# mjrgh/DCSExplorer

Hardware: AMD Instinct MI355X
Metric: bit_exact_int16_pcm_samples_per_sec (higher is better)
Workload: dtype int16; 1 GPU; survey3_65536; gpu_max_hw_queues=4, samples_per_frame=240, frames_per_wave=8, wavefronts_per_launch=8192, arithmetic=ADSP-2105 1.15 fixed point, 32-bit integer intermediates, partition=range over streams, no collective, scale=1, inflight=1, frames_per_chunk=all, full=False

## Files before the change

### dcsexplorer_amd/csrc/dcs_decode_chunk.inc.h

```cpp
    DCS_STAMP(1);

    struct { uint32_t job; uint32_t prevSlot, flags, nSrc, shiftXform; uint32_t firstSrc, prevJob, poolOff, bpl; } slot;
    uint32_t exportNext;
    uint4 pd0, pd1, phdr;
    uint2 pd2;
    uint32_t planHdr0 = 0, planHdr1 = 0, planType0 = 0, planType1 = 0;
    {
        uint4 *scratch = reinterpret_cast<uint4 *>(L.pool());
        static_assert(kHeadVec * 16 <= poolDwords(FPW) * 4, "the package head fits in the bit pool");
        if (lane < kHeadVec)
            scratch[lane] = phead0;
        if (kHeadLoads > 1 && lane + 64 < kHeadVec)
            scratch[lane + 64] = phead1;
        waveSync();
        const uint4 *sp5 = scratch + 5 * s;
        const uint4 s0 = sp5[0];
        pd0 = sp5[1]; pd1 = sp5[2];
        const uint4 d2v = sp5[3];
        pd2 = make_uint2(d2v.x, d2v.y);
        phdr = sp5[4];
        if constexpr (bandPlanInLds(FPW))
        {
            const unsigned char *bytes = reinterpret_cast<const unsigned char *>(sp5) + q;
            planType0 = bytes[36]; planType1 = bytes[44];
// ... 166 lines not shown
                const uint32_t hw = static_cast<uint32_t>((streamOff + 2) >> 2);
                const uint32_t sh = static_cast<uint32_t>((streamOff + 2) & 3);
                uint32_t hdrW[5];
#pragma unroll
                for (int i = 0 ; i < 5 ; ++i)
                    hdrW[i] = (has && hw + i < blobWords) ? blobW[hw + i] : 0u;
                Q.h0 = __builtin_amdgcn_alignbyte(hdrW[1], hdrW[0], sh);
                Q.h1 = __builtin_amdgcn_alignbyte(hdrW[2], hdrW[1], sh);
                Q.h2 = __builtin_amdgcn_alignbyte(hdrW[3], hdrW[2], sh);
                Q.h3 = __builtin_amdgcn_alignbyte(hdrW[4], hdrW[3], sh);
                if (hdrLen == 1)
                {
                    Q.h0 &= 0xFFu; Q.h1 = Q.h2 = Q.h3 = 0;
                }
            }
            waveSync();

            if (R0) DCS_STAMP(3);
            const bool ok = has && fits && unpacker;
            if (has && !fits && q == 0)
                err |= DCS_FRAME_FATAL | DCS_FRAME_STOP;
            if (has && q == 0)
                err |= flags >> 4;
            uint32_t relBits = hdrBits;
            Q.bandBase = 0;
            Q.outIdx = 1;
            Q.prv = 0; Q.prvDelta = 0;
            Q.subType = (format == DCS_FMT_93B_T1) ? 0 : 2;
            Q.reuse = false; Q.first = true;
            Q.midEnd = Q.midStart = Q.midStraddle = false;
            Q.endIdx = 0;
            constexpr bool evenDeal = R0 && SUB == 8 && EVEN;
            if (serial)
                Q.nb = (q == 0) ? nBands : 0;
            else
            {
                const int nb16 = min(nBands, 16);
                if (R0)
                {
                    const bool f93a = format == DCS_FMT_93A_T1;
                    const int nbEnd = f93a ? min(nBands, 18) : nb16;
                    const int myBase = (sp.x & 0x8000u) ? nbEnd
                                     : static_cast<int>(sp.y >> 28) + ((f93a && (sp.y & (DCS_SPLIT_BASE16 << 16)) != 0) ? 16 : 0);
                    const int nextBase = __shfl(myBase, lane + FPW);
                    Q.bandBase = myBase;
                    Q.nb = max((q == SUB - 1 ? nbEnd : nextBase) - myBase, 0);
                    if (SUB == 16)
                    {
                        const bool mid = format >= DCS_FMT_94_T0 && q == SUB - 1 && myBase == 15 && (sp.y & (DCS_SPLIT_MID15 << 16)) != 0;
                        const bool nextMid = __shfl(static_cast<int>(mid), lane + FPW) != 0;
                        Q.midStart = mid;
                        Q.midStraddle = mid && (sp.y & (DCS_MID15_STRADDLE << 16)) != 0;
                        Q.midEnd = q == SUB - 2 && nextMid;
                        if (Q.midEnd)
                            Q.nb = 16 - myBase;
                    }
                    if constexpr (evenDeal)
                    {
                        const bool mid = format >= DCS_FMT_94_T0 && !(sp.x & 0x8000u) && (sp.y & (DCS_SPLIT_MID15 << 16)) != 0;
                        const bool nextMid = __shfl(static_cast<int>(mid), lane + FPW) != 0 && q != SUB - 1;
                        const int nextIdx = __shfl(static_cast<int>((sp.y >> 16) & 0x1FFu), lane + FPW);
                        Q.midStart = mid;
                        Q.midStraddle = mid && (sp.y & (DCS_MID15_STRADDLE << 16)) != 0;
                        Q.midEnd = nextMid;
                        Q.endIdx = nextIdx;
                        if (nextMid)
                            Q.nb = min(nextBase + 1, nbEnd) - myBase;
                    }
                }
                else
                {
                    const int bpl = max((nb16 + SUB - 1) / SUB, 1);
                    if (format == DCS_FMT_93A_T1)
                    {
                        Q.bandBase = min(q * bpl, nb16);
                        Q.nb = min(max(nb16 - Q.bandBase, 0), bpl);
                    }
                    else
                    {
                        Q.bandBase = dcsLaneFirstBand(format, q, bpl, nb16);
                        Q.nb = (q == SUB - 1 ? nb16 : dcsLaneFirstBand(format, q + 1, bpl, nb16)) - Q.bandBase;
                    }
                }
                if (q != 0 && Q.nb != 0)
                {
                    if (!R0)
                        sp = reinterpret_cast<const uint2 *>(sdp)[5 + Q.bandBase - 1];
                    const uint32_t sp0 = sp.x, sp1 = sp.y;
                    relBits = sp0 & 0x7FFFu;
                    Q.prv = sp0 >> 16;
                    Q.prvDelta = sp1 & 0xFFFFu;
                    const uint32_t st = sp1 >> 16;
                    Q.outIdx = static_cast<int>(st & 0x1FFu);
                    Q.subType = static_cast<int>((st >> 9) & 3u);
                    Q.reuse = (st & 0x800u) != 0;
                    Q.first = false;
                }
            }
            const uint32_t inPool = static_cast<uint32_t>(bitPos & 31) + relBits;
            const uint32_t *brAt = pool + (ok ? off + (inPool >> 5) : 0u);
            const int brBit = static_cast<int>(inPool & 31);

            if (R0) DCS_STAMP(12);
            const bool is94 = ok && format >= DCS_FMT_94_T0;
            const bool is93a = ok && format == DCS_FMT_93A_T1 && Q.nb != 0 && !(Q.bandBase != 0 && Q.reuse);
            const bool is93 = ok && format < DCS_FMT_93A_T1;
            if (__any(is94))
            {
                BR94 br;
                br.init(brAt, brBit);
                const uint32_t planAt = (R0 && bandPlanInLds(FPW))
                    ? static_cast<uint32_t>(reinterpret_cast<uintptr_t>((LdsBytePtr)L.plan())) + static_cast<uint32_t>(Q.bandBase * FPW + s) * kPlanRecBytes
                    : 0u;
                err |= unpack94<R0, BR94, SUB, evenDeal>(T, row, br, Q, format, mixMul, is94, stamp, planAt);
            }
            if constexpr (!SOLE)
            {
            BR93 br;
            br.init(brAt, brBit);
            if (__any(is93))
                err |= unpack93<R0, BR93>(T, row, br, Q, format, mixMul, is93, stamp);
            if (is93a)
            {
                constexpr bool kSpreadTail = SUB == 16 && !R0;
                const int end = Q.bandBase + Q.nb;
                const int end2 = (!R0 && SUB != 16 && end >= 16 && nBands > 16) ? nBands : end;
                const int prv0 = Q.bandBase == 0 ? 0x1A : sx16(Q.prv), out0 = Q.bandBase == 0 ? 0 : Q.outIdx;
                const int hb0 = static_cast<int>(Q.h0 & 0xFFu);
                if (pairTableInLds(FPW))
                    err |= unpack93a<R0, BR93>(T, row, br, hb0, mixMul, reinterpret_cast<const uint16_t *>(smem + ldsBytes(FPW) - 4096),
                                         Q.bandBase, end2, prv0, out0);
                else
                    err |= unpack93a<R0, BR93>(T, row, br, hb0, mixMul, a.tables->pair93a, Q.bandBase, end2, prv0, out0);
                if (kSpreadTail && pairTableInLds(FPW) && q < 2 && 16 + q < nBands)
                {
                    const uint32_t r0 = q == 0 ? Q.t0 : Q.t2, r1 = q == 0 ? Q.t1 : Q.t3;
                    if (!((r1 >> 16) & 0x800u))
                    {
                        const uint32_t inPool2 = static_cast<uint32_t>(bitPos & 31) + (r0 & 0xFFFFu);
                        BR93 br2;
                        br2.init(pool + off + (inPool2 >> 5), static_cast<int>(inPool2 & 31));
                        err |= unpack93a<R0, BR93>(T, row, br2, hb0, mixMul, reinterpret_cast<const uint16_t *>(smem + ldsBytes(FPW) - 4096),
                                             16 + q, 17 + q, sx16(r0 >> 16), static_cast<int>((r1 >> 16) & 0x1FFu));
                    }
                }
            }
            }
            waveSync();
        };

        {
            if (__any(myNSrc > 0))
                unpackRound(std::true_type{}, 0);
            if constexpr (!SOLE)
                for (int r = 1 ; __any(r < myNSrc) ; ++r)
                    unpackRound(std::false_type{}, r);
        }

        DCS_STAMP(4);
        if (__any(err != 0))
        {
#pragma unroll
            for (int m = FPW ; m < 64 ; m <<= 1)
                err |= __shfl_xor(err, m);
        }
        if (live && q == 0)
        {
            if constexpr (!SOLE)
                if (job.xform == DCS_XFORM_93)
                    dcMagnitude93(row);
            if (!(slot.flags & DCS_SLOT_HALO) && a.err != nullptr)
                a.err[slot.job] = err;
        }
    }
    waveSync();

    DCS_STAMP(5);
    uint32_t *tails = reinterpret_cast<uint32_t *>(L.tails());
#ifdef DCS_STAMPS
    asm volatile("s_waitcnt vmcnt(0)" ::: "memory");
    DCS_STAMP(7);
#endif
    const int nSlots = __popcll(__ballot(live && lane < FPW));
    const int slotJob = static_cast<int>(slot.job);
    const int slotWord = static_cast<int>(slot.flags | (slot.prevSlot << 8) | (static_cast<uint32_t>(job.volShift) << 16));
    const int jobXform = job.xform, jobPrev = static_cast<int>(job.prev);


    constexpr bool kOnePass = SOLE;
    static_assert(!kOnePass || (EVEN && FPW == 8), "the even deal: 8 frames per wavefront, one transform pass of 8");
    const unsigned long long slots94 = kOnePass ? 0ull : __ballot(live && lane < FPW && jobXform == DCS_XFORM_94);
    const bool oneXform = kOnePass || slots94 == 0 || slots94 == __ballot(live && lane < FPW);
    for (int s0 = 0 ; kOnePass || s0 < nSlots ; )
    {
        const int xf = kOnePass ? DCS_XFORM_94 : __builtin_amdgcn_readlane(jobXform, s0);
        const int G = (xf == DCS_XFORM_94) ? 8 : 4;
#ifndef DCS_RUN_BALLOT_MIN_FPW
#define DCS_RUN_BALLOT_MIN_FPW 8
#endif
        int n = 1;
        if constexpr (kOnePass)
            n = nSlots;
        else if constexpr (FPW >= DCS_RUN_BALLOT_MIN_FPW)
        {
            const unsigned long long sameXf = (xf == DCS_XFORM_94) ? slots94 : ~slots94;
            n = min(min(static_cast<int>(__builtin_ctzll(~(sameXf >> s0))), G), nSlots - s0);
        }
        else if (oneXform)
            n = min(G, nSlots - s0);
        else
        {
            while (n < G && s0 + n < nSlots && __builtin_amdgcn_readlane(jobXform, s0 + n) == xf)
                ++n;
        }

        if constexpr (!kOnePass)
            if (xf != constsXform)
            {
                constsXform = xf;
                loadLaneConsts(a.tables, lane, constsXform, C);
            }
        const int lpfShift = (xf == DCS_XFORM_94) ? 3 : 4;
        const int g = lane >> lpfShift;
        const bool active = g < n;
        const int mySlot = s0 + (active ? g : 0);
        const int myWord = __shfl(slotWord, mySlot);
        const int myFlags = myWord & 0xFF, myPrevSlot = (myWord >> 8) & 0xFF, myShift = myWord >> 16;
        const uint32_t myJob = static_cast<uint32_t>(__shfl(slotJob, mySlot));
        const uint32_t myPrevJob = static_cast<uint32_t>(__shfl(jobPrev, mySlot));
        const int lr = (xf == DCS_XFORM_94) ? bitrevN(lane & 7, 3) : bitrevN(lane & 15, 4);

        uint32_t extTail = 0;
        if (__any(active && (myFlags & DCS_SLOT_EXT_TAIL) != 0))
        {
            if (active && (myFlags & DCS_SLOT_EXT_TAIL) != 0 && a.tailsIn != nullptr)
            {
                const size_t k = static_cast<size_t>(myPrevJob & 0x7FFFFFFFu);
                extTail = (xf == DCS_XFORM_94) ? reinterpret_cast<const uint32_t *>(a.tailsIn)[k * 8 + lr]
                                               : static_cast<uint32_t>(static_cast<uint16_t>(a.tailsIn[k * 16 + lr]));
            }
        }

        PassLane P;
        P.rowC = active ? reinterpret_cast<uint32_t *>(L.row(mySlot)) : L.pool();
#ifdef DCS_STAMPS_XFORM
        P.stamp = stamp;
#endif
        P.l = lane & ((1 << lpfShift) - 1);
        P.shiftPair = static_cast<uint32_t>(myShift) * 0x00010001u;
        P.paced = paced && kPace.steps && s0 + n >= nSlots;

        uint32_t x[16];
        BflyRegs R;
        R.k8000 = 0x8000u; R.k10000 = 0x10000u; R.watch = 0xFFFFu;
        R.k4000 = 0x4000u; R.watchB = 0x7FFF7FFFu;
        asm volatile("" : "+v"(R.k8000), "+v"(R.k10000), "+v"(R.k4000));
        if constexpr (kOnePass)
            transform94x8<kPace.levels, true>(P, W, C, R, x, 16u - ((a.flags >> DCS_BATCH_BANDS_SHIFT) & DCS_BATCH_BANDS_MASK));
        else if (xf == DCS_XFORM_94)
            transform94x8<kPace.levels>(P, W, C, R, x);
        else
            transform93x4<kPace.levels>(P, W, C, R, x);
        if (s0 == 0) DCS_STAMP(14);

        {
            const int ts = active ? mySlot : FPW;
            if (xf == DCS_XFORM_94)
                tails[ts * 8 + lr] = x[15];
            else
                reinterpret_cast<uint16_t *>(tails)[ts * 16 + lr] = static_cast<uint16_t>(x[15]);
        }
        waveSync();

        if (s0 == 0) DCS_STAMP(15);
        const bool emit = active && !(myFlags & DCS_SLOT_HALO);
        const bool hasPrev = myPrevSlot != DCS_NO_PREV_SLOT;
        const bool exporter = active && (myFlags & DCS_SLOT_EXPORT) != 0;
        const bool deferred = active && (myFlags & DCS_SLOT_IMPORT) != 0;
#ifndef DCS_RDV_SPLIT_FPW4
#define DCS_RDV_SPLIT_FPW4 12
#endif
        constexpr int kSplit = FPW == 4 ? DCS_RDV_SPLIT_FPW4 : 8;
        int lrA = lr;
        if (FPW == 4)
            asm volatile("" : "+v"(lrA));
        unsigned long long metAsProducer = 0, metAsConsumer = 0;
        auto rendezvous = [&](uint32_t mine0, uint32_t tailOut)
        {
            if (exporter)
                metAsProducer = __hip_atomic_exchange(a.handoff + static_cast<size_t>(chunk) * 16 + lrA, handoffWord(a.epoch, 0u, tailOut),
                                                      __ATOMIC_RELAXED, __HIP_MEMORY_SCOPE_AGENT);
            if (deferred)
                metAsConsumer = __hip_atomic_exchange(a.handoff + static_cast<size_t>(myPrevJob) * 16 + lrA, handoffWord(a.epoch, 1u, mine0),
                                                      __ATOMIC_RELAXED, __HIP_MEMORY_SCOPE_AGENT);
        };
        if (kOnePass || xf == DCS_XFORM_94)
        {
            uint32_t tailPair = tails[(hasPrev ? myPrevSlot : mySlot) * 8 + lr];
            tailPair = hasPrev ? tailPair : extTail;
            const uint32_t mixed = packC(overlapMix(reC(x[0]), C.k[DCS_K94_OVLA] & 0xFFFFu, reC(tailPair), C.k[DCS_K94_OVLB] & 0xFFFFu),
                                         overlapMix(imC(x[0]), C.k[DCS_K94_OVLA] >> 16, imC(tailPair), C.k[DCS_K94_OVLB] >> 16));
            x[0] = deferred ? x[0] : mixed;
            uint32_t *out = reinterpret_cast<uint32_t *>(a.pcm) + static_cast<size_t>(myJob) * (DCS_FRAME_SAMPLES / 2) + lrA;
            if (emit)
            {
                if (!deferred)
                    out[0] = x[0];
#pragma unroll
                for (int r = 1 ; r < kSplit ; ++r)
                    out[8 * bitrevN(r, 4)] = x[r];
            }
            rendezvous(x[0], x[15]);
            if (emit)
            {
#pragma unroll
                for (int r = kSplit ; r < 15 ; ++r)
                    out[8 * bitrevN(r, 4)] = x[r];
                if (a.tailsOut != nullptr && (myFlags & DCS_SLOT_KEEP_TAIL))
                    reinterpret_cast<uint32_t *>(a.tailsOut)[static_cast<size_t>(myJob) * 8 + lrA] = x[15];
            }
            if (deferred && handoffMeets(metAsConsumer, a.epoch, 0u))
            {
                const uint32_t theirTail = static_cast<uint32_t>(metAsConsumer);
                out[0] = packC(overlapMix(reC(x[0]), C.k[DCS_K94_OVLA] & 0xFFFFu, reC(theirTail), C.k[DCS_K94_OVLB] & 0xFFFFu),
                               overlapMix(imC(x[0]), C.k[DCS_K94_OVLA] >> 16, imC(theirTail), C.k[DCS_K94_OVLB] >> 16));
            }
            if (exporter && handoffMeets(metAsProducer, a.epoch, 1u))
            {
                const uint32_t theirs = static_cast<uint32_t>(metAsProducer);
                reinterpret_cast<uint32_t *>(a.pcm)[static_cast<size_t>(exportNext) * (DCS_FRAME_SAMPLES / 2) + lrA] =
                    packC(overlapMix(reC(theirs), C.k[DCS_K94_OVLA] & 0xFFFFu, reC(x[15]), C.k[DCS_K94_OVLB] & 0xFFFFu),
                          overlapMix(imC(theirs), C.k[DCS_K94_OVLA] >> 16, imC(x[15]), C.k[DCS_K94_OVLB] >> 16));
            }
        }
        else if constexpr (!kOnePass)
        {
            int tailSample = static_cast<int16_t>(reinterpret_cast<const uint16_t *>(tails)[(hasPrev ? myPrevSlot : mySlot) * 16 + lr]);
            tailSample = hasPrev ? tailSample : sx16(extTail);
            const uint32_t mixed = static_cast<uint32_t>(overlapMix(reC(x[0]), C.k[DCS_K93_OVL] & 0xFFFFu, tailSample, C.k[DCS_K93_OVL] >> 16)) & 0xFFFFu;
            x[0] = deferred ? (x[0] & 0xFFFFu) : mixed;
            int16_t *out = a.pcm + static_cast<size_t>(myJob) * DCS_FRAME_SAMPLES + lrA;
            if (emit)
            {
                if (!deferred)
                    out[0] = static_cast<int16_t>(x[0]);
#pragma unroll
                for (int r = 1 ; r < kSplit ; ++r)
                    out[16 * bitrevN(r, 4)] = static_cast<int16_t>(x[r]);
            }
            rendezvous(x[0], x[15] & 0xFFFFu);
            if (emit)
            {
#pragma unroll
                for (int r = kSplit ; r < 15 ; ++r)
                    out[16 * bitrevN(r, 4)] = static_cast<int16_t>(x[r]);
                if (a.tailsOut != nullptr && (myFlags & DCS_SLOT_KEEP_TAIL))
                    a.tailsOut[static_cast<size_t>(myJob) * 16 + lrA] = static_cast<int16_t>(x[15]);
            }
            if (deferred && handoffMeets(metAsConsumer, a.epoch, 0u))
                out[0] = static_cast<int16_t>(overlapMix(reC(x[0]), C.k[DCS_K93_OVL] & 0xFFFFu, sx16(static_cast<uint32_t>(metAsConsumer)), C.k[DCS_K93_OVL] >> 16));
            if (exporter && handoffMeets(metAsProducer, a.epoch, 1u))
                a.pcm[static_cast<size_t>(exportNext) * DCS_FRAME_SAMPLES + lrA] =
                    static_cast<int16_t>(overlapMix(reC(static_cast<uint32_t>(metAsProducer)), C.k[DCS_K93_OVL] & 0xFFFFu, sx16(x[15]), C.k[DCS_K93_OVL] >> 16));
        }
        waveSync();
        s0 += n;
        if constexpr (kOnePass)
            break;
    }

    DCS_STAMP(6);
```

### dcsexplorer_amd/csrc/dcs_kernels.hip.h

```cpp
#pragma once
#include <hip/hip_runtime.h>
#include <type_traits>
#include <cstddef>
#include "dcs_common.h"

namespace dcsk {

struct Stamper
{
#ifdef DCS_STAMPS
    unsigned long long *p;
#ifdef DCS_STAMPS_REALTIME
    __device__ __forceinline__ void operator()(int k) const { if (p != nullptr) p[k] = __builtin_amdgcn_s_memrealtime(); }
#else
    __device__ __forceinline__ void operator()(int k) const { if (p != nullptr) p[k] = __builtin_amdgcn_s_memtime(); }
#endif
#else
    __device__ __forceinline__ void operator()(int) const { }
#endif
};
#define DCS_STAMP(k) stamp(k)

__device__ __forceinline__ unsigned long long handoffWord(uint32_t epoch, uint32_t who, uint32_t payload)
{
// ... 690 lines not shown
{
    const int p = __mul24(a, b);
    uint32_t mr = (static_cast<uint32_t>(p) << 1) + 0x8000u;
    if ((p & 0x7FFF) == 0x4000)
        mr &= ~0x10000u;
    return mr;
}

__device__ __forceinline__ void dcMagnitude93(uint16_t *row)
{
    const uint32_t w = *reinterpret_cast<const uint32_t *>(row);
    const int f0 = sx16(w), f1 = static_cast<int>(w) >> 16;
    const bool neg = f0 < 0;
    const int a0 = sx16(static_cast<uint32_t>(neg ? -f0 : f0));
    uint32_t sr = prodSS(f1, f1) + prodSS(a0, a0);
    int exponent = calcExp32(sr);
    sr <<= -exponent;
    const int x = sx16(sr >> 16);
    uint32_t mr = 0x0D490000u;
    mr += static_cast<uint32_t>(0x5D1D * x) << 1;
    int mf = static_cast<int>(mulRound(x, x)) >> 16;
    mr += static_cast<uint32_t>(-22035 * mf) << 1;
    mf = static_cast<int>(mulRound(x, mf)) >> 16;
    mr += static_cast<uint32_t>(0x46D6 * mf) << 1;
    mf = static_cast<int>(mulRound(x, mf)) >> 16;
    mr += static_cast<uint32_t>(-8790 * mf) << 1;
    mf = static_cast<int>(mulRound(x, mf)) >> 16;
    mr += static_cast<uint32_t>(0x072D * mf) << 1;
    const bool odd = (exponent & 1) != 0;
    const uint32_t mrOdd = mulRound(static_cast<int>(mr) >> 16, 0x5A82);
    mr = odd ? mrOdd : mr;
    exponent = ((exponent + (odd ? 1 : 0)) >> 1) + 1;
    const uint32_t up = mr << (exponent & 31);
    const uint32_t down = static_cast<uint32_t>(static_cast<int>(mr) >> ((-exponent) & 31));
    uint32_t ar = (exponent >= 0 ? up : down) >> 16;
    ar = neg ? static_cast<uint32_t>(-sx16(ar)) & 0xFFFFu : ar;
    ar = x != 0 ? ar : 0u;
    *reinterpret_cast<uint32_t *>(row) = ar;
}

typedef short s16x2 __attribute__((ext_vector_type(2)));
typedef unsigned short u16x2 __attribute__((ext_vector_type(2)));

__device__ __forceinline__ uint32_t pkAddSat(uint32_t a, uint32_t b)
{ return __builtin_bit_cast(uint32_t, __builtin_elementwise_add_sat(__builtin_bit_cast(s16x2, a), __builtin_bit_cast(s16x2, b))); }
__device__ __forceinline__ uint32_t pkSubSat(uint32_t a, uint32_t b)
{ return __builtin_bit_cast(uint32_t, __builtin_elementwise_sub_sat(__builtin_bit_cast(s16x2, a), __builtin_bit_cast(s16x2, b))); }
__device__ __forceinline__ uint32_t pkAdd(uint32_t a, uint32_t b)
{ return __builtin_bit_cast(uint32_t, static_cast<u16x2>(__builtin_bit_cast(u16x2, a) + __builtin_bit_cast(u16x2, b))); }
__device__ __forceinline__ uint32_t pkSub(uint32_t a, uint32_t b)
{ return __builtin_bit_cast(uint32_t, static_cast<u16x2>(__builtin_bit_cast(u16x2, a) - __builtin_bit_cast(u16x2, b))); }
__device__ __forceinline__ uint32_t pkAshr(uint32_t a, uint32_t shiftPair)
{ return __builtin_bit_cast(uint32_t, static_cast<s16x2>(__builtin_bit_cast(s16x2, a) >> __builtin_bit_cast(s16x2, shiftPair))); }

__device__ __forceinline__ uint32_t packC(int re, int im) { return (static_cast<uint32_t>(re) & 0xFFFFu) | (static_cast<uint32_t>(im) << 16); }
__device__ __forceinline__ int reC(uint32_t c) { return sx16(c); }
__device__ __forceinline__ int imC(uint32_t c) { return static_cast<int>(c) >> 16; }

__device__ __forceinline__ void quirkWatch(uint32_t &watch, uint32_t a, uint32_t b)
{
    asm("v_min_u16 %0, %0, %1\n\tv_min_u16 %0, %0, %2" : "+v"(watch) : "v"(a), "v"(b));
}
__device__ __forceinline__ bool quirkSeen(uint32_t watch) { return __any((watch & 0xFFFFu) == 0); }
#define DCS_MUL_SEL(dst, x, xsel, y, ysel) \
    asm("v_mul_i32_i24_sdwa %0, sext(%1), sext(%2) dst_sel:DWORD dst_unused:UNUSED_PAD src0_sel:" xsel " src1_sel:" ysel : "=v"(dst) : "v"(x), "v"(y))

struct BflyRegs
{
    uint32_t k8000, k10000; uint32_t watch;
    uint32_t k4000, watchB;
};

struct TwScalar { int c2, s2, ns2; };
struct TwA { TwScalar t[8]; };
constexpr int kTwADoubled[8][2] = { { -65536, 0 }, { 0, -65536 }, { -46340, -46340 }, { 46340, -46340 },
                                    { -60548, -25080 }, { 25080, -60548 }, { -25080, -60548 }, { 60548, -25080 } };
__device__ __forceinline__ void loadTwA(const DcsDevTables *, TwA &W)
{
#pragma unroll
    for (int k = 2 ; k < 8 ; ++k)
        W.t[k] = TwScalar{ kTwADoubled[k][0], kTwADoubled[k][1], -kTwADoubled[k][1] };
}

__device__ __forceinline__ uint32_t rotateExact(uint32_t A, int c, int s)
{
    const int are = reC(A), aim = imC(A);
    const int p2 = __mul24(aim, s);
    const int dR = __mul24(are, c) - p2;
    const int q2 = __mul24(are, s);
    const int dI = __mul24(aim, c) + q2;
    uint32_t mrR = (static_cast<uint32_t>(dR) << 1) + 0x8000u;
    uint32_t mrI = (static_cast<uint32_t>(dI) << 1) + 0x8000u;
    if ((p2 & 0x7FFF) == 0x4000) mrR &= ~0x10000u;
    if ((q2 & 0x7FFF) == 0x4000) mrI &= ~0x10000u;
    return __builtin_amdgcn_perm(mrI, mrR, 0x07060302u);
}

__device__ __forceinline__ uint32_t rotateFastA(uint32_t A, const TwScalar &t, BflyRegs &R)
{
    const int are = reC(A), aim = imC(A);
    const uint32_t nP = static_cast<uint32_t>(__mul24(aim, t.ns2)) + R.k8000;
    const uint32_t mrR = static_cast<uint32_t>(__mul24(are, t.c2)) + nP;
    const uint32_t qK = static_cast<uint32_t>(__mul24(are, t.s2)) + R.k8000;
    const uint32_t mrI = static_cast<uint32_t>(__mul24(aim, t.c2)) + qK;
    quirkWatch(R.watch, nP, qK);
    return __builtin_amdgcn_perm(mrI, mrR, 0x07060302u);
}
__device__ __forceinline__ uint32_t shl1Add(uint32_t a, uint32_t b)
{
    uint32_t r = (a << 1) + b;
    asm("" : "+v"(r));
    return r;
}
template <bool TIGHT>
__device__ __forceinline__ uint32_t rotateFastB(uint32_t A, uint32_t tw, BflyRegs &R)
{
    int p1, p2, q1, q2;
    DCS_MUL_SEL(p2, A, "WORD_1", tw, "WORD_1");
    DCS_MUL_SEL(p1, A, "WORD_0", tw, "WORD_0");
    DCS_MUL_SEL(q2, A, "WORD_0", tw, "WORD_1");
    DCS_MUL_SEL(q1, A, "WORD_1", tw, "WORD_0");
    if (TIGHT)
    {
        const uint32_t tR = shl1Add(static_cast<uint32_t>(p2), R.k8000);
        const uint32_t mrR = shl1Add(static_cast<uint32_t>(p1), R.k10000) - tR;
        const uint32_t qK = shl1Add(static_cast<uint32_t>(q2), R.k8000);
        const uint32_t mrI = shl1Add(static_cast<uint32_t>(q1), qK);
        quirkWatch(R.watch, tR, qK);
        return __builtin_amdgcn_perm(mrI, mrR, 0x07060302u);
    }
    const uint32_t mrR = (static_cast<uint32_t>(p1 - p2) << 1) + R.k8000;
    const uint32_t qK = (static_cast<uint32_t>(q2) << 1) + R.k8000;
    const uint32_t mrI = (static_cast<uint32_t>(q1) << 1) + qK;
    quirkWatch(R.watch, (static_cast<uint32_t>(p2) << 1) + R.k8000, qK);
    return __builtin_amdgcn_perm(mrI, mrR, 0x07060302u);
}

struct TwDot { uint32_t re, im, s2; };
__device__ __forceinline__ TwDot deriveTwDot(uint32_t tw)
{
    TwDot d;
    d.im = __builtin_amdgcn_alignbit(tw, tw, 16);
    d.re = __builtin_bit_cast(uint32_t, static_cast<u16x2>(__builtin_bit_cast(u16x2, tw) * __builtin_bit_cast(u16x2, 0xFFFF0001u)));
    asm("v_pk_add_u16 %0, %1, %1 op_sel:[1,1] op_sel_hi:[1,1]" : "=v"(d.s2) : "v"(tw));
    return d;
}
template <bool FIX>
__device__ __forceinline__ uint32_t rotateDotB(uint32_t A, const TwDot &t, BflyRegs &R, uint32_t fixMask)
{
    uint32_t xR, xI, lows;
    const uint32_t cR = FIX ? ((A & fixMask) | R.k4000) : R.k4000;
    asm("v_dot2_i32_i16 %0, %1, %2, %3" : "=v"(xR) : "v"(A), "v"(t.re), "v"(cR));
    asm("v_dot2_i32_i16 %0, %1, %2, %3" : "=v"(xI) : "v"(A), "v"(t.im), "v"(R.k4000));
    asm("v_pk_mul_lo_u16 %0, %1, %2" : "=v"(lows) : "v"(A), "v"(t.s2));
    asm("v_pk_min_i16 %0, %0, %1" : "+v"(R.watchB) : "v"(lows));
    return __builtin_amdgcn_perm(xI << 1, xR << 1, 0x07060302u);
}
__device__ __forceinline__ bool quirkSeenB(uint32_t w) { return __any((w & 0xFFFFu) == 0x8000u || (w >> 16) == 0x8000u); }

template <bool SAT>
__device__ __forceinline__ void addSub(uint32_t u, uint32_t T, uint32_t &lo, uint32_t &hi)
{
    if (SAT) { lo = pkSubSat(u, T); hi = pkAddSat(u, T); }
    else     { lo = pkSub(u, T);    hi = pkAdd(u, T); }
}

__device__ __forceinline__ uint32_t rotateByMinusOne(uint32_t A) { return pkSub(0u, A); }
__device__ __forceinline__ uint32_t rotateByMinusI(uint32_t A)
{
    return __builtin_bit_cast(uint32_t, static_cast<u16x2>(__builtin_bit_cast(u16x2, __builtin_amdgcn_alignbit(A, A, 16))
                                                            * __builtin_bit_cast(u16x2, 0xFFFF0001u)));
}

template <bool SAT, int D, int SH>
__device__ __forceinline__ void stageA(uint32_t (&x)[16], const TwA &W, BflyRegs &R)
{
    uint32_t y[16];
#pragma unroll
    for (int r = 0 ; r < 16 ; ++r)
        if (!(r & D))
        {
            const int idx = r >> SH;
            const uint32_t T = idx == 0 ? rotateByMinusOne(x[r + D]) : idx == 1 ? rotateByMinusI(x[r + D])
                                                                                 : rotateFastA(x[r + D], W.t[idx], R);
            addSub<SAT>(x[r], T, y[r], y[r + D]);
        }
    if (__builtin_expect(quirkSeen(R.watch), 0))
    {
        R.watch = 0xFFFFu;
#pragma unroll
        for (int r = 0 ; r < 16 ; ++r)
            if (!(r & D) && (r >> SH) >= 2)
            {
                int c2 = W.t[r >> SH].c2, s2 = W.t[r >> SH].s2;
                asm volatile("" : "+v"(c2), "+v"(s2));
                addSub<SAT>(x[r], rotateExact(x[r + D], c2 >> 1, s2 >> 1), y[r], y[r + D]);
            }
    }
#pragma unroll
    for (int r = 0 ; r < 16 ; ++r)
        x[r] = y[r];
}
template <bool SAT, int D, int SH, bool DOT = !SAT>
__device__ __forceinline__ void stageB(uint32_t (&x)[16], const uint32_t *tw, BflyRegs &R)
{
    uint32_t y[16];
    bool redo;
    if constexpr (DOT)
    {
        constexpr int kTw = 8 / D;
        TwDot td[kTw];
#pragma unroll
        for (int k = 0 ; k < kTw ; ++k)
            td[k] = deriveTwDot(tw[k]);
        constexpr int kFix = kTw == 1 ? 0 : 1;
        const uint32_t fixMask = tw[kFix] == 0x80000000u ? 0xFFFF0000u : 0u;
#pragma unroll
        for (int r = 0 ; r < 16 ; ++r)
            if (!(r & D))
            {
                const uint32_t T = (r >> SH) == kFix ? rotateDotB<true>(x[r + D], td[r >> SH], R, fixMask)
                                                     : rotateDotB<false>(x[r + D], td[r >> SH], R, 0u);
                addSub<SAT>(x[r], T, y[r], y[r + D]);
            }
        redo = quirkSeenB(R.watchB);
        if (redo)
            R.watchB = 0x7FFF7FFFu;
    }
    else
    {
#pragma unroll
        for (int r = 0 ; r < 16 ; ++r)
            if (!(r & D))
                addSub<SAT>(x[r], rotateFastB<SAT>(x[r + D], tw[r >> SH], R), y[r], y[r + D]);
        redo = quirkSeen(R.watch);
        if (redo)
            R.watch = 0xFFFFu;
    }
    if (__builtin_expect(redo, 0))
    {
#pragma unroll
        for (int r = 0 ; r < 16 ; ++r)
            if (!(r & D))
                addSub<SAT>(x[r], rotateExact(x[r + D], sx16(tw[r >> SH]), static_cast<int>(tw[r >> SH]) >> 16), y[r], y[r + D]);
    }
#pragma unroll
    for (int r = 0 ; r < 16 ; ++r)
        x[r] = y[r];
}

__device__ __forceinline__ int bitrev9(int v) { return static_cast<int>(__brev(static_cast<uint32_t>(v)) >> 23); }
__device__ __forceinline__ int bitrevN(int v, int bits) { return static_cast<int>(__brev(static_cast<uint32_t>(v)) >> (32 - bits)); }

__device__ __forceinline__ int overlapMix(int x, uint32_t cx, int o, uint32_t co)
{
    const uint32_t a = static_cast<uint32_t>(x * static_cast<int>(cx)) << 1;
    const uint32_t b = static_cast<uint32_t>(o * static_cast<int>(co)) << 1;
    return static_cast<int>(a + b + 0x8000u) >> 16;
}

typedef uint32_t u32x4a4 __attribute__((ext_vector_type(4), aligned(4)));

struct LaneConsts { uint32_t k[DCS_LANE_CONSTS]; };
__device__ __forceinline__ void loadLaneConsts(const DcsDevTables *G, int lane, int xform, LaneConsts &C)
{
    const uint4 *src = reinterpret_cast<const uint4 *>(xform == DCS_XFORM_94 ? G->lane94[lane] : G->lane93[lane]);
#pragma unroll
    for (int i = 0 ; i < DCS_LANE_CONSTS / 4 ; ++i)
    {
        const uint4 v = src[i];
        C.k[4 * i] = v.x; C.k[4 * i + 1] = v.y; C.k[4 * i + 2] = v.z; C.k[4 * i + 3] = v.w;
    }
}

__device__ __forceinline__ void waveSync()
{
    __builtin_amdgcn_fence(__ATOMIC_RELEASE, "wavefront");
    __builtin_amdgcn_wave_barrier();
    __builtin_amdgcn_fence(__ATOMIC_ACQUIRE, "wavefront");
}

struct PassLane
{
    uint32_t *rowC;
    int l;
    uint32_t shiftPair;
    bool paced;
#ifdef DCS_STAMPS_XFORM
    Stamper stamp;
#endif
};
constexpr int kPaceSteps = 2 | (1 << 2) | (0 << 4);
#define DCS_PACE_STEP(k) do { if (P.paced) __builtin_amdgcn_s_setprio((STEPS >> (2 * (k))) & 3); } while (0)
#ifdef DCS_STAMPS_XFORM
#define DCS_XSTAMP(k) P.stamp(k)
#else
#define DCS_XSTAMP(k)
#endif

__device__ __forceinline__ uint4 ldsRead4(const uint32_t *p) { return *reinterpret_cast<const uint4 *>(p); }
__device__ __forceinline__ void ldsWrite4(uint32_t *p, uint32_t a, uint32_t b, uint32_t c, uint32_t d)
{ *reinterpret_cast<uint4 *>(p) = make_uint4(a, b, c, d); }

__device__ __forceinline__ int swzQuad(int row, int quad) { return row * 16 + ((quad ^ (row >> 1)) & 3) * 4; }
__device__ __forceinline__ int swzPos(int row, int pos) { return swzQuad(row, pos >> 2) + (pos & 3); }

template <int STEPS, bool SHORT = false>
__device__ __forceinline__ void transform94x8(const PassLane &P, const TwA &W, const LaneConsts &C, BflyRegs &R, uint32_t (&x)[16],
                                              uint32_t maxBands = 16)
{
    const int l = P.l;
    uint32_t *S = P.rowC;
    uint32_t An[8], Bn[8];
    {
        uint32_t a_[8], b_[8];
        auto head = [&](auto zjTag)
        {
            constexpr int ZJ = decltype(zjTag)::value;
#pragma unroll
            for (int j = 0 ; j < 8 ; ++j)
            {
                const int i = l + 8 * j;
                const uint32_t X = P.rowC[i];
                if (j < ZJ)
                {
                    a_[j] = b_[j] = pkSub(0u, X);
                    continue;
                }
                uint32_t Y = P.rowC[(128 - i) & 127];
                if (i == 0) Y = 0;
                const uint32_t Sm = pkAddSat(X, Y), Df = pkSubSat(X, Y);
                a_[j] = pkSub(0u, __builtin_amdgcn_perm(Df, Sm, 0x07060100u));
                b_[j] = pkSub(0u, __builtin_amdgcn_perm(Sm, Df, 0x07060100u));
            }
        };
        if constexpr (SHORT)
        {
            static_assert(dcsPrepassShort(dcsPrepassBands(5)) >= 5 && dcsPrepassShort(dcsPrepassBands(3)) >= 3, "the short forms' band counts");
            if (maxBands <= static_cast<uint32_t>(dcsPrepassBands(5)))
                head(std::integral_constant<int, 5>());
            else if (maxBands <= static_cast<uint32_t>(dcsPrepassBands(3)))
                head(std::integral_constant<int, 3>());
            else
                head(std::integral_constant<int, 0>());
        }
        else
            head(std::integral_constant<int, 0>());
        auto finish = [&](int j, uint32_t Pr)
        {
            const uint32_t a = a_[j];
            An[j] = pkAddSat(Pr, a);
            const uint32_t t = pkSubSat(a, Pr);
            const uint32_t t2 = pkSubSat(Pr, a);
            Bn[j] = __builtin_amdgcn_perm(t2, t, 0x07060100u);
        };
#pragma unroll
        for (int j = 0 ; j < 8 ; ++j)
        {
            int p1, p2, q1, q2;
            DCS_MUL_SEL(p2, b_[j], "WORD_0", C.k[DCS_K94_PRE + j], "WORD_0");
            DCS_MUL_SEL(p1, b_[j], "WORD_1", C.k[DCS_K94_PRE + j], "WORD_1");
            DCS_MUL_SEL(q2, b_[j], "WORD_0", C.k[DCS_K94_PRE + j], "WORD_1");
            DCS_MUL_SEL(q1, b_[j], "WORD_1", C.k[DCS_K94_PRE + j], "WORD_0");
            const uint32_t tR = shl1Add(static_cast<uint32_t>(p2), R.k8000);
            const uint32_t m0 = shl1Add(static_cast<uint32_t>(p1), R.k10000) - tR;
            const uint32_t qK = shl1Add(static_cast<uint32_t>(q2), R.k8000);
            const uint32_t m1 = shl1Add(static_cast<uint32_t>(q1), qK);
            quirkWatch(R.watch, tR, qK);
            finish(j, __builtin_amdgcn_perm(m0, m1, 0x07060302u));
        }
        if (__builtin_expect(quirkSeen(R.watch), 0))
        {
            R.watch = 0xFFFFu;
#pragma unroll
            for (int j = 0 ; j < 8 ; ++j)
            {
                const int b0 = reC(b_[j]), b1 = imC(b_[j]);
                const int c0 = sx16(C.k[DCS_K94_PRE + j]), c1 = static_cast<int>(C.k[DCS_K94_PRE + j]) >> 16;
                const int p2 = __mul24(b0, c0), q2 = __mul24(b0, c1);
                uint32_t m0 = (static_cast<uint32_t>(__mul24(b1, c1) - p2) << 1) + 0x8000u;
                uint32_t m1 = (static_cast<uint32_t>(__mul24(b1, c0) + q2) << 1) + 0x8000u;
                if ((p2 & 0x7FFF) == 0x4000) m0 &= ~0x10000u;
                if ((q2 & 0x7FFF) == 0x4000) m1 &= ~0x10000u;
                finish(j, __builtin_amdgcn_perm(m0, m1, 0x07060302u));
            }
        }
    }
    if (l == 0)
    {
        const uint32_t M = P.rowC[64];
        Bn[0] = __builtin_amdgcn_perm(M, pkSub(0u, M), 0x07060100u);
    }
    waveSync();
    {
        ldsWrite4(S + swzQuad(l, 0), An[0], An[1], An[2], An[3]);
        ldsWrite4(S + swzQuad(l, 1), An[4], An[5], An[6], An[7]);
        const int rb = (8 - l) & 7;
        if (l != 0)
        {
            ldsWrite4(S + swzQuad(rb, 2), Bn[7], Bn[6], Bn[5], Bn[4]);
            ldsWrite4(S + swzQuad(rb, 3), Bn[3], Bn[2], Bn[1], Bn[0]);
        }
        else
        {
            ldsWrite4(S + swzQuad(rb, 2), Bn[0], Bn[7], Bn[6], Bn[5]);
            ldsWrite4(S + swzQuad(rb, 3), Bn[4], Bn[3], Bn[2], Bn[1]);
        }
    }
    waveSync();
#pragma unroll
    for (int c = 0 ; c < 4 ; ++c)
    {
        const uint4 v = ldsRead4(S + swzQuad(l, c));
        x[4 * c] = v.x; x[4 * c + 1] = v.y; x[4 * c + 2] = v.z; x[4 * c + 3] = v.w;
    }
    waveSync();
    DCS_PACE_STEP(0);
#pragma unroll
    for (int r = 0 ; r < 8 ; ++r)
    {
        const uint32_t u = x[r], a = x[r + 8];
        x[r] = pkAddSat(u, a); x[r + 8] = pkSubSat(u, a);
    }
    stageA<true, 4, 3>(x, W, R);
    stageA<true, 2, 2>(x, W, R);
    stageA<true, 1, 1>(x, W, R);
    DCS_PACE_STEP(1);
#pragma unroll
    for (int r = 0 ; r < 16 ; ++r)
        S[swzPos(r >> 1, 8 * (r & 1) + l)] = x[r];
    waveSync();
#pragma unroll
    for (int c = 0 ; c < 4 ; ++c)
    {
        const uint4 v = ldsRead4(S + swzQuad(l, c));
        x[4 * c] = v.x; x[4 * c + 1] = v.y; x[4 * c + 2] = v.z; x[4 * c + 3] = v.w;
    }
    stageB<true, 4, 3>(x, C.k + DCS_K94_TWB, R);
    DCS_PACE_STEP(2);
    stageB<true, 2, 2>(x, C.k + DCS_K94_TWB + 2, R);
    stageB<true, 1, 1>(x, C.k + DCS_K94_TWB + 6, R);
    if (__any(P.shiftPair != 0))
    {
#pragma unroll
        for (int r = 0 ; r < 16 ; ++r)
            x[r] = pkAshr(x[r], P.shiftPair);
    }
}

template <int STEPS>
__device__ __forceinline__ void transform93x4(const PassLane &P, const TwA &W, const LaneConsts &C, BflyRegs &R, uint32_t (&x)[16])
{
    const int l = P.l;
    uint32_t *S = P.rowC;
#pragma unroll
    for (int r = 0 ; r < 8 ; ++r)
    {
        const int p = 16 * r + l;
        const uint32_t A = P.rowC[p];
        const uint32_t B = P.rowC[(128 - p) & 127];
        const uint32_t Sm = pkAdd(A, B), Df = pkSub(A, B);
        x[r] = __builtin_amdgcn_perm(Df, Sm, 0x07060100u);
        x[r + 8] = __builtin_amdgcn_perm(Sm, Df, 0x07060100u);
        if (p == 0)
        {
            x[0] = A; x[8] = A;
        }
    }
    DCS_XSTAMP(8);
    DCS_PACE_STEP(0);
    stageA<false, 4, 3>(x, W, R);
    stageA<false, 2, 2>(x, W, R);
    stageA<false, 1, 1>(x, W, R);
    DCS_XSTAMP(9);
    waveSync();
    uint32_t y[16];
#pragma unroll
    for (int h = 0 ; h < 2 ; ++h)
    {
#pragma unroll
        for (int r = 0 ; r < 8 ; ++r)
            S[swzPos(r, l)] = x[8 * h + r];
        waveSync();
        if ((l >> 3) == h)
        {
#pragma unroll
            for (int c = 0 ; c < 4 ; ++c)
            {
                const uint4 v = ldsRead4(S + swzQuad(l & 7, c));
                y[4 * c] = v.x; y[4 * c + 1] = v.y; y[4 * c + 2] = v.z; y[4 * c + 3] = v.w;
            }
        }
        waveSync();
    }
#pragma unroll
    for (int r = 0 ; r < 16 ; ++r)
        x[r] = y[r];
    DCS_XSTAMP(10);
    DCS_PACE_STEP(1);
    stageB<false, 8, 4>(x, C.k + DCS_K93_TWB, R);
    stageB<false, 4, 3>(x, C.k + DCS_K93_TWB + 1, R);
    DCS_PACE_STEP(2);
    stageB<false, 2, 2>(x, C.k + DCS_K93_TWB + 3, R);
    stageB<false, 1, 1>(x, C.k + DCS_K93_TWB + 7, R);
    DCS_XSTAMP(11);
    if (__any(P.shiftPair != 0))
    {
#pragma unroll
        for (int r = 0 ; r < 16 ; ++r)
            x[r] = pkAshr(x[r], P.shiftPair);
    }
}

#ifndef DCS_CPW2_SCHED
#define DCS_CPW2_SCHED 1
#endif
struct PaceSchedule { int entry; bool steps; int levels; };
__host__ __device__ constexpr PaceSchedule paceSchedule(int cpw, int pass)
{
    if (cpw == 1)
        return { 3, true, kPaceSteps };
#if DCS_CPW2_SCHED == 0
    return pass == 0 ? PaceSchedule{ 3, false, kPaceSteps } : PaceSchedule{ 3, true, 2 | (1 << 2) | (0 << 4) };
#elif DCS_CPW2_SCHED == 1
    return pass == 0 ? PaceSchedule{ 3, false, kPaceSteps } : PaceSchedule{ 2, true, 1 | (1 << 2) | (0 << 4) };
#elif DCS_CPW2_SCHED == 2
    return pass == 0 ? PaceSchedule{ 3, true, 3 | (3 << 2) | (2 << 4) } : PaceSchedule{ 2, true, 1 | (1 << 2) | (0 << 4) };
#else
    return pass == 0 ? PaceSchedule{ 3, true, 3 | (2 << 2) | (2 << 4) } : PaceSchedule{ 1, true, 1 | (0 << 2) | (0 << 4) };
#endif
}

template <int FPW, int CPW = 1, bool EVEN = false, bool SOLE = false>
#ifndef DCS_MIN_WAVES
#define DCS_MIN_WAVES 4
#endif
__global__ void __launch_bounds__(64 * kWavesPerBlock, DCS_MIN_WAVES)
dcsDecodeKernel(uint8_t *kPackages, const DcsDevTables *kTables, uint32_t kNChunks, uint32_t kFlags, uint32_t kEpoch, uint32_t kNJobs,
                int16_t *kPcm, unsigned long long *kHandoff, uint32_t *kErr, int16_t *kTailsOut,
                const uint8_t *kBlob, uint64_t kBlobLen, const DcsSrcDesc *kSrcs, const int16_t *kTailsIn, unsigned long long *kDebug)
{
    DcsKernelArgs a;
    a.blob = kBlob; a.blobLen = kBlobLen; a.srcs = kSrcs; a.packages = kPackages; a.nChunks = kNChunks; a.nJobs = kNJobs;
    a.pcm = kPcm; a.err = kErr; a.tailsIn = kTailsIn; a.tailsOut = kTailsOut; a.tables = kTables; a.debug = kDebug;
    a.handoff = kHandoff; a.epoch = kEpoch; a.flags = kFlags;
    extern __shared__ __attribute__((aligned(16))) unsigned char smem[];
    const int wave = static_cast<int>(threadIdx.x) >> 6;
    const int lane = static_cast<int>(threadIdx.x) & 63;
    constexpr int kPoolBytes = poolDwords(FPW) * 4, kTileBytes = waveTileBytes(FPW);
    static_assert(kPoolBytes % 16 == 0 && kWavesPerBlock * kTileBytes >= 8192, "LDS layout");
    const Lds<FPW> L{ smem, smem + DCS_LDS_DECODE_BYTES + kWavesPerBlock * kPoolBytes + wave * kTileBytes,
                      smem + DCS_LDS_DECODE_BYTES + wave * kPoolBytes };
    uint32_t blk = blockIdx.x;
    if (a.flags & DCS_BATCH_XCD_RANGES)
        blk = (blk & 7u) * (gridDim.x >> 3) + (blk >> 3);
    static_assert(CPW == 1 || CPW == 2, "one or two chunks per wavefront");
    static_assert((!EVEN || FPW == 8) && (!SOLE || EVEN), "the even deal: 8 frames per wavefront; SOLE: an even-deal kernel");
    const uint32_t wv = blk * kWavesPerBlock + static_cast<uint32_t>(wave);
    const uint32_t nFirst = CPW == 2 ? (a.nChunks + 1u) >> 1 : a.nChunks;
    auto stamperOf = [&](uint32_t chunk, bool valid)
    {
#ifdef DCS_STAMPS
        return Stamper{ (lane == 0 && a.debug != nullptr && valid) ? a.debug + static_cast<size_t>(chunk) * 16 : nullptr };
#else
        return Stamper{};
#endif
    };
    {
        const Stamper stamp = stamperOf(wv, wv < nFirst);
        DCS_STAMP(0);
    }
    const bool pacedLaunch = (a.flags & DCS_BATCH_PACED) != 0;
    const bool paced = pacedLaunch && blockIdx.x + ((a.flags >> DCS_BATCH_CUS8_SHIFT) & 0xFFu) * 32u >= gridDim.x;
    if (pacedLaunch) __builtin_amdgcn_s_setprio(3);
    constexpr int SUB = subLanes(FPW);
#ifndef DCS_DIRECT_MAX_FPW
#define DCS_DIRECT_MAX_FPW 4
#endif
    using BR94 = typename std::conditional<(FPW <= DCS_DIRECT_MAX_FPW), DirectReader, BitReader>::type;
    using BR93 = DirectReader;
    static_assert(SUB * FPW == 64 && SUB <= 16, "every lane unpacks; a frame has at most 16 split lanes");
    const int s = lane % FPW;
    const int q = lane / FPW;
    const bool unpacker = q < SUB;

    const uint32_t layout = (a.flags >> DCS_BATCH_IMG_SHIFT) & DCS_BATCH_IMG_MASK;
    const int imgDw = static_cast<int>(dcsPkgImgDw(layout));
    const bool split4 = (layout & DCS_PKG_SPLIT4) != 0;
    const uint32_t offPool = split4 ? dcsPkgOffPool(FPW, DCS_PKG_SPLIT4) : dcsPkgOffPool(FPW, 0);
    constexpr int kHeadVec = FPW * 5, kHeadLoads = (kHeadVec + 63) / 64;
    static_assert(kHeadLoads <= 2, "package head: two 16-byte loads per lane at most");
    uint4 phead0, phead1 = make_uint4(0, 0, 0, 0);
    uint2 psplit;
    constexpr int kPoolPieces = (poolDwords(FPW) + 255) / 256;
    uint4 pimg[kPoolPieces];
    {
        const uint32_t chunk = wv;
        const bool valid = wv < nFirst;
#include "dcs_request_package.inc.h"
    }
    TwA W;
    loadTwA(a.tables, W);

    {
        constexpr int kTableVec = DCS_LDS_DECODE_BYTES / 16;
        static_assert(kTableVec <= 64 * kWavesPerBlock, "one piece of the tables per thread");
// ... 79 lines not shown
```

Measured before the change: 577.8 billion samples/s.

## Stage PCM output through LDS and emit coalesced 16-byte stores in sole mode

In the SOLE path, each lane now writes its bit-reversed transform outputs into the per-frame LDS row instead of scattering 4-byte global stores. It also stores the job id and flags beside them. After a wave sync, lanes read contiguous 16-byte pieces across all frames and write them with dwordx4 global stores using an inline-asm store with the sc1 cache hint. The aim is to replace strided scalar stores with coalesced wide ones. The cost is an extra LDS round trip and a sync, and the halo/import masking logic must stay correct.

```diff
diff --git a/dcsexplorer_amd/csrc/dcs_decode_chunk.inc.h b/dcsexplorer_amd/csrc/dcs_decode_chunk.inc.h
--- a/dcsexplorer_amd/csrc/dcs_decode_chunk.inc.h
+++ b/dcsexplorer_amd/csrc/dcs_decode_chunk.inc.h
@@ -492,22 +492,59 @@
                                          overlapMix(imC(x[0]), C.k[DCS_K94_OVLA] >> 16, imC(tailPair), C.k[DCS_K94_OVLB] >> 16));
             x[0] = deferred ? x[0] : mixed;
             uint32_t *out = reinterpret_cast<uint32_t *>(a.pcm) + static_cast<size_t>(myJob) * (DCS_FRAME_SAMPLES / 2) + lrA;
-            if (emit)
-            {
+            if constexpr (SOLE)
+            {
+                uint32_t *rowO = P.rowC + lrA;
                 if (!deferred)
-                    out[0] = x[0];
-#pragma unroll
-                for (int r = 1 ; r < kSplit ; ++r)
-                    out[8 * bitrevN(r, 4)] = x[r];
-            }
-            rendezvous(x[0], x[15]);
-            if (emit)
-            {
-#pragma unroll
-                for (int r = kSplit ; r < 15 ; ++r)
-                    out[8 * bitrevN(r, 4)] = x[r];
-                if (a.tailsOut != nullptr && (myFlags & DCS_SLOT_KEEP_TAIL))
+                    rowO[0] = x[0];
+#pragma unroll
+                for (int r = 1 ; r < 15 ; ++r)
+                    rowO[8 * bitrevN(r, 4)] = x[r];
+                if (P.l == 0)
+                    *reinterpret_cast<uint2 *>(P.rowC + 130) = make_uint2(myJob, static_cast<uint32_t>(myFlags));
+                waveSync();
+                rendezvous(x[0], x[15]);
+                U32x4 piece[4];
+                char *dst[4];
+                bool put[4];
+#pragma unroll
+                for (int t = 0 ; t < 4 ; ++t)
+                {
+                    const int g = lane + 64 * t;
+                    const int f = min((g * 2185) >> 16, FPW - 1), p = g - 30 * f;
+                    const uint32_t *rowF = reinterpret_cast<const uint32_t *>(L.row(f));
+                    const uint2 jf = *reinterpret_cast<const uint2 *>(rowF + 130);
+                    const uint4 v = ldsRead4(rowF + 4 * (p & 31));
+                    piece[t] = U32x4{ v.x, v.y, v.z, v.w };
+                    put[t] = g < 240 && f < nSlots && !(jf.y & DCS_SLOT_HALO) && !((jf.y & DCS_SLOT_IMPORT) != 0 && p < 2);
+                    dst[t] = reinterpret_cast<char *>(a.pcm) + static_cast<size_t>(jf.x) * (DCS_FRAME_SAMPLES * 2) + p * 16;
+                }
+#pragma unroll
+                for (int t = 0 ; t < 4 ; ++t)
+                    if (put[t])
+                        storePcm16(dst[t], piece[t]);
+                if (emit && a.tailsOut != nullptr && (myFlags & DCS_SLOT_KEEP_TAIL))
                     reinterpret_cast<uint32_t *>(a.tailsOut)[static_cast<size_t>(myJob) * 8 + lrA] = x[15];
+            }
+            else
+            {
+                if (emit)
+                {
+                    if (!deferred)
+                        out[0] = x[0];
+#pragma unroll
+                    for (int r = 1 ; r < kSplit ; ++r)
+                        out[8 * bitrevN(r, 4)] = x[r];
+                }
+                rendezvous(x[0], x[15]);
+                if (emit)
+                {
+#pragma unroll
+                    for (int r = kSplit ; r < 15 ; ++r)
+                        out[8 * bitrevN(r, 4)] = x[r];
+                    if (a.tailsOut != nullptr && (myFlags & DCS_SLOT_KEEP_TAIL))
+                        reinterpret_cast<uint32_t *>(a.tailsOut)[static_cast<size_t>(myJob) * 8 + lrA] = x[15];
+                }
             }
             if (deferred && handoffMeets(metAsConsumer, a.epoch, 0u))
             {
diff --git a/dcsexplorer_amd/csrc/dcs_kernels.hip.h b/dcsexplorer_amd/csrc/dcs_kernels.hip.h
--- a/dcsexplorer_amd/csrc/dcs_kernels.hip.h
+++ b/dcsexplorer_amd/csrc/dcs_kernels.hip.h
@@ -1016,6 +1016,12 @@
 __device__ __forceinline__ void ldsWrite4(uint32_t *p, uint32_t a, uint32_t b, uint32_t c, uint32_t d)
 { *reinterpret_cast<uint4 *>(p) = make_uint4(a, b, c, d); }
 
+typedef uint32_t U32x4 __attribute__((ext_vector_type(4)));
+__device__ __forceinline__ void storePcm16(void *p, U32x4 v)
+{
+    asm volatile("global_store_dwordx4 %0, %1, off sc1\n\ts_nop 0" : : "v"(p), "v"(v) : "memory");
+}
+
 __device__ __forceinline__ int swzQuad(int row, int quad) { return row * 16 + ((quad ^ (row >> 1)) & 3) * 4; }
 __device__ __forceinline__ int swzPos(int row, int pos) { return swzQuad(row, pos >> 2) + (pos & 3); }
 
```

Result: faster. 617.5 billion samples/s (median of 6 runs) (+6.9%).
